# LinXueyuanStdio/LaTeX_OCR

Hardware: NVIDIA H100
Metric: formula-images/sec (train step, 128x512 px, seq<=150) (higher is better)
Workload: dtype bf16

## Files before the change

latex_ocr_b200/csrc/lo_attention.cu:

```cuda
#include <cooperative_groups.h>

#include <mutex>
#include <vector>

#include "lo_common.cuh"
#include "lo_ptx.cuh"

namespace cg = cooperative_groups;

namespace lo {

#ifndef LO_ATT_RPW
#define LO_ATT_RPW 2
#endif
#ifndef LO_ATT_MINB
#define LO_ATT_MINB 2
#endif
#define AP_THREADS 288
#define AP_CWARPS 8
#define AP_STAGES 3
#define AP_MAXSPLIT 16


#ifdef LO_ATT_TIMING
__device__ long long* g_att_ts = nullptr;
__device__ __forceinline__ void att_ts(int k) {
  if (g_att_ts) {
    long long t;
    asm volatile("mov.u64 %0, %%globaltimer;" : "=l"(t));
    g_att_ts[((int64_t)blockIdx.y * gridDim.x + blockIdx.x) * 16 + k] = t;
  }
}
#define ATT_TS(k, cond) do { if (cond) att_ts(k); } while (0)
#else
#define ATT_TS(k, cond) do { } while (0)
#endif

__host__ __device__ __forceinline__ bool att_keep_stage(int i, int depth, int keep_q) {
  const int j = i - depth;
  return j >= 0 && (((j + 1) * keep_q) >> 10) != ((j * keep_q) >> 10);
}

template <int ACT, bool APPROX>
__device__ __forceinline__ float att_act(float x) {
  if constexpr (ACT == 0) return fmaxf(x, 0.f);
  else if constexpr (APPROX) {
    float y;
    asm("tanh.approx.f32 %0, %1;" : "=f"(y) : "f"(x));
    return y;
  } else return tanhf(x);
}
template <int ACT>
__device__ __forceinline__ float att_dact(float pre, float post) {
  if constexpr (ACT == 0) return pre > 0.f ? 1.f : 0.f;
  else return 1.f - post * post;
}

__host__ __device__ __forceinline__ int att_rows_per_split(int R, int nsplit) { return (((R + nsplit - 1) / nsplit) + 1) & ~1; }

template <typename T, int NVA, int NVC>
struct ApCfg {
  static constexpr int CHA = NVA * 256;
  static constexpr int CHC = NVC * 256;
  static constexpr int NVM = NVA > NVC ? NVA : NVC;
  static constexpr int RPW = (sizeof(T) == 2 && NVM <= 2) ? LO_ATT_RPW : 1;
  static constexpr int ROWS = AP_CWARPS * RPW;
  static constexpr int HALF_A = ROWS * CHA;
  static constexpr int HALF_C = ROWS * CHC;
  static constexpr int STAGE_ELEMS = HALF_A + HALF_C;
  static constexpr int STAGE_BYTES = STAGE_ELEMS * (int)sizeof(T);
  static constexpr int SMEM = AP_STAGES * STAGE_BYTES + 128;
};

template <typename T, int NVA, int NVC, bool CL, int ACT, bool MK>
__device__ __forceinline__ void attention_fwd_pipe_cta(
    const T* __restrict__ att1, const T* __restrict__ enc, const float* __restrict__ att2, int64_t att2_stride,
    const float* __restrict__ wf, float* __restrict__ alpha, int64_t alpha_stride, float* __restrict__ ctx,
    float* __restrict__ gate_pre, int64_t gate_stride, float* __restrict__ gctx, bf16* __restrict__ gctx_bf, int R, int nsplit,
    int* __restrict__ counters, float* __restrict__ partials, int keep_q, uint8_t* __restrict__ mask_out, int b, int sp, int64_t g0,
    int64_t pbase) {
  using C = ApCfg<T, NVA, NVC>;
  constexpr int CHA = C::CHA, CHC = C::CHC;
  extern __shared__ __align__(128) uint8_t ap_smem[];
  T* ring = reinterpret_cast<T*>(ap_smem);
  uint64_t* full_bar = reinterpret_cast<uint64_t*>(ap_smem + AP_STAGES * C::STAGE_BYTES);
  uint64_t* empty_bar = full_bar + AP_STAGES;
  float* s_e = reinterpret_cast<float*>(ap_smem + AP_STAGES * C::STAGE_BYTES + 128);
  __shared__ float s_m[AP_CWARPS], s_l[AP_CWARPS];
  __shared__ float s_msplit[AP_MAXSPLIT], s_lsplit[AP_MAXSPLIT];
  __shared__ int s_last;

  const int lane = threadIdx.x & 31, wid = threadIdx.x >> 5;
  const int rps = (R + nsplit - 1) / nsplit;
  const int r0 = sp * rps, r1 = min(R, r0 + rps);
  const int nst = r1 > r0 ? (r1 - r0 + C::ROWS - 1) / C::ROWS : 0;
  const T* a1b = att1 + g0 * CHA;
  const T* eb = enc + g0 * CHC;
  float* alb = alpha + (int64_t)b * alpha_stride;
  ATT_TS(0, threadIdx.x == 0);

  if (threadIdx.x == 0) {
    for (int s = 0; s < AP_STAGES; s++) {
      mbar_init(full_bar + s, 1);
      mbar_init(empty_bar + s, AP_CWARPS);
    }
    fence_barrier_init();
  }
  __syncthreads();
  float m = -INFINITY, l = 0.f;
  float gate_pf = 0.f;
  float acc[NVC * 8];
#pragma unroll
  for (int i = 0; i < NVC * 8; i++) acc[i] = 0.f;

  if (wid == AP_CWARPS) {
    if (lane == 0) {
      const uint64_t pk = l2_policy_evict_normal(), ps = l2_policy_evict_first();
      for (int i = 0; i < nst; i++) {
        const int s = i % AP_STAGES;
        const uint32_t ph = (i / AP_STAGES) & 1;
        mbar_wait(empty_bar + s, ph ^ 1);
        const int row = r0 + i * C::ROWS;
        const int rows = min(C::ROWS, r1 - row);
        const uint32_t bytes_a = (uint32_t)rows * CHA * (uint32_t)sizeof(T), bytes_c = (uint32_t)rows * CHC * (uint32_t)sizeof(T);
        T* sa = ring + (size_t)s * C::STAGE_ELEMS;
        const uint64_t pol = att_keep_stage(i, AP_STAGES, keep_q) ? pk : ps;
        mbar_expect_tx(full_bar + s, bytes_a + bytes_c);
        ATT_TS(6, i == 0);
        ATT_TS(7, i == nst - 1);
        bulk_g2s(sa, a1b + (int64_t)row * CHA, bytes_a, full_bar + s, pol);
        bulk_g2s(sa + C::HALF_A, eb + (int64_t)row * CHC, bytes_c, full_bar + s, pol);
      }
    }
    __syncwarp();
    pdl_wait();
  } else {
    float a2[NVA * 8], wv[NVA * 8];
#pragma unroll
    for (int j = 0; j < NVA; j++) ld8(wf + (j * 32 + lane) * 8, wv + j * 8);
    pdl_wait();
    ATT_TS(1, threadIdx.x == 0);
    pdl_trigger();
#pragma unroll
    for (int j = 0; j < NVA; j++) ld8(att2 + (int64_t)b * att2_stride + (j * 32 + lane) * 8, a2 + j * 8);
    if (CL && gate_pre && (int)threadIdx.x < (CHC + nsplit - 1) / nsplit && sp * ((CHC + nsplit - 1) / nsplit) + (int)threadIdx.x < CHC)
      gate_pf = gate_pre[(int64_t)b * gate_stride + sp * ((CHC + nsplit - 1) / nsplit) + threadIdx.x];
    ATT_TS(2, threadIdx.x == 0);
    for (int i = 0; i < nst; i++) {
      const int s = i % AP_STAGES;
// ... 126 lines not shown
        Lg += ml[1] * scl[q];
      }
    }
    const float invL = 1.0f / Lg;
    const int cps = (CHC + nsplit - 1) / nsplit;
    for (int c = sp * cps + threadIdx.x; c < min(CHC, (sp + 1) * cps); c += AP_THREADS) {
      float t = 0.f;
#pragma unroll
      for (int q = 0; q < 8; q++)
        if (q < nsplit) t = fmaf(cluster.map_shared_rank(s_part, q)[c], scl[q], t);
      t *= invL;
      ctx[(int64_t)b * CHC + c] = t;
      if (gate_pre) {
        const bool pf = c == sp * cps + (int)threadIdx.x && (int)threadIdx.x < AP_CWARPS * 32;
        const float g = sigmoidf_(pf ? gate_pf : gate_pre[(int64_t)b * gate_stride + c]);
        gate_pre[(int64_t)b * gate_stride + c] = g;
        gctx[(int64_t)b * CHC + c] = g * t;
        if (gctx_bf) gctx_bf[(int64_t)b * CHC + c] = __float2bfloat16_rn(g * t);
      } else if (gctx_bf) {
        gctx_bf[(int64_t)b * CHC + c] = __float2bfloat16_rn(t);
      }
    }
    for (int r = r0 + threadIdx.x; r < r1; r += AP_THREADS) alb[r] = expf(s_e[r - r0] - Mg) * invL;
    cluster.sync();
    ATT_TS(5, threadIdx.x == 0);
    return;
  }
  float* part = partials + (pbase + sp) * (CHC + 2);
  for (int c = threadIdx.x; c < CHC; c += AP_THREADS) {
    float t = 0.f;
#pragma unroll
    for (int w = 0; w < AP_CWARPS; w++) t = fmaf(s_acc[w * CHC + c], wsc[w], t);
    part[2 + c] = t;
  }
  if (threadIdx.x == 0) { part[0] = M; part[1] = L; }
  __threadfence();
  __syncthreads();
  if (threadIdx.x == 0) {
    const int ticket = atomicAdd(counters + b, 1);
    s_last = (ticket == nsplit - 1);
    if (s_last) counters[b] = 0;
  }
  __syncthreads();
  if (!s_last) {
    ATT_TS(5, threadIdx.x == 0);
    return;
  }
  __threadfence();
  ATT_TS(9, threadIdx.x == 0);
  const float* pb = partials + pbase * (CHC + 2);
  constexpr int PS = 8;
  constexpr int RB = 4;
  if ((int)threadIdx.x < nsplit) {
    s_msplit[threadIdx.x] = __ldcg(pb + (int64_t)threadIdx.x * (CHC + 2));
    s_lsplit[threadIdx.x] = __ldcg(pb + (int64_t)threadIdx.x * (CHC + 2) + 1);
  }
  float pv[PS], ev[RB];
  auto load_parts = [&](int c) {
#pragma unroll
    for (int s = 0; s < PS; s++) pv[s] = s < nsplit ? __ldcg(pb + (int64_t)s * (CHC + 2) + 2 + c) : 0.f;
  };
  if ((int)threadIdx.x < CHC) load_parts(threadIdx.x);
#pragma unroll
  for (int k = 0; k < RB; k++) {
    const int r = threadIdx.x + k * AP_THREADS;
    ev[k] = r < R ? __ldcg(alb + r) : 0.f;
// ... 24 lines not shown
        const float g = sigmoidf_(gpf[k]);
        gate_pre[(int64_t)b * gate_stride + c] = g;
        gctx[(int64_t)b * CHC + c] = g * t;
        if (gctx_bf) gctx_bf[(int64_t)b * CHC + c] = __float2bfloat16_rn(g * t);
      } else if (gctx_bf) {
        gctx_bf[(int64_t)b * CHC + c] = __float2bfloat16_rn(t);
      }
    }
  }
#pragma unroll
  for (int k = 0; k < RB; k++) {
    const int r = threadIdx.x + k * AP_THREADS;
    if (r < R) alb[r] = expf(ev[k] - Mg) * invL;
  }
  for (int r = threadIdx.x + RB * AP_THREADS; r < R; r += AP_THREADS) alb[r] = expf(__ldcg(alb + r) - Mg) * invL;
  ATT_TS(5, threadIdx.x == 0);
}

template <typename T, int NVA, int NVC, bool CL, int ACT, bool MK>
__global__ void __launch_bounds__(AP_THREADS, LO_ATT_MINB) attention_fwd_pipe_kernel(
    const T* __restrict__ att1, const T* __restrict__ enc, const float* __restrict__ att2, int64_t att2_stride,
    const float* __restrict__ wf, float* __restrict__ alpha, int64_t alpha_stride, float* __restrict__ ctx,
    float* __restrict__ gate_pre, int64_t gate_stride, float* __restrict__ gctx, bf16* __restrict__ gctx_bf, int R, int nsplit,
    int* __restrict__ counters, float* __restrict__ partials, int keep_q, int rpi, uint8_t* __restrict__ mask_out) {
  const int b = blockIdx.y, sp = blockIdx.x;
  attention_fwd_pipe_cta<T, NVA, NVC, CL, ACT, MK>(att1, enc, att2, att2_stride, wf, alpha, alpha_stride, ctx, gate_pre, gate_stride, gctx,
                                                  gctx_bf, R, nsplit, counters, partials, keep_q, mask_out, b, sp,
                                                  (int64_t)(b / rpi) * R, (int64_t)b * nsplit);
}

template <typename T, int NVA, int NVC>
__global__ void __launch_bounds__(AP_THREADS, LO_ATT_MINB) attention_fwd_ragged_kernel(
    const T* __restrict__ att1, const T* __restrict__ enc, const float* __restrict__ att2, int64_t att2_stride,
    const float* __restrict__ wf, float* __restrict__ alpha, int64_t alpha_stride, float* __restrict__ ctx,
    float* __restrict__ gate_pre, int64_t gate_stride, float* __restrict__ gctx, bf16* __restrict__ gctx_bf,
    const int4* __restrict__ cta_map, const int32_t* __restrict__ reg_off, int rpi, int* __restrict__ counters,
    float* __restrict__ partials, int keep_q) {
  const int4 e = cta_map[blockIdx.x];
  const int img = e.x / rpi;
  const int g0 = reg_off[img];
  attention_fwd_pipe_cta<T, NVA, NVC, false, 0, false>(att1, enc, att2, att2_stride, wf, alpha, alpha_stride, ctx, gate_pre, gate_stride,
                                                      gctx, gctx_bf, reg_off[img + 1] - g0, e.z, counters, partials, keep_q, nullptr,
                                                      e.x, e.y, (int64_t)g0, (int64_t)e.w);
}

__host__ __device__ __forceinline__ int att_ragged_row_splits(int ns, int B, int Ri, int64_t sumR, bool fixed) {
  if (fixed) return ns;
  const int64_t q = (int64_t)ns * B * Ri / sumR;
  return q < 1 ? 1 : (q > AP_MAXSPLIT ? AP_MAXSPLIT : (int)q);
}

__global__ void attention_ragged_map_kernel(const int32_t* __restrict__ reg_off, int B, int rpi, int ns, int64_t sumR, int fixed,
                                            int4* __restrict__ cta_map, int* __restrict__ counters) {
  extern __shared__ int s_rows[];
  for (int b = threadIdx.x; b < B; b += blockDim.x) {
    s_rows[b] = att_ragged_row_splits(ns, B, reg_off[b / rpi + 1] - reg_off[b / rpi], sumR, fixed != 0);
    counters[b] = 0;
  }
  __syncthreads();
  if (threadIdx.x == 0) {
    int p = 0;
    for (int b = 0; b < B; b++) {
      s_rows[B + b] = p;
      p += s_rows[b];
    }
  }
// ... 562 lines not shown
  }
  float macc[4][4];
#pragma unroll
  for (int j = 0; j < 4; j++)
#pragma unroll
    for (int i = 0; i < 4; i++) macc[j][i] = 0.f;

  if (wid == AP_CWARPS) {
    const uint64_t pk = l2_policy_evict_normal(), pm = l2_policy_evict_first();
    for (int i = 0; i < nst; i++) {
      const int s = i % ABM_STAGES;
      const uint32_t ph = (i / ABM_STAGES) & 1;
      const int row = r0 + i * ABM_ROWS;
      const int rows = min(ABM_ROWS, r1 - row);
      const uint32_t bytes_m = (uint32_t)((rows + 1) >> 1) * 2u * MB;
      uint8_t* st = ap_smem + (size_t)s * ABM_STAGE_BYTES;
      if (lane == 0) {
        mbar_wait(empty_bar + s, ph ^ 1);
        mbar_expect_tx(full_bar + s, (uint32_t)rows * CH * 2u + bytes_m);
        ATT_TS(6, i == 0);
        ATT_TS(7, i == nst - 1);
      }
      __syncwarp();
      const uint64_t pe = att_keep_stage(i, ABM_STAGES, keep_q) ? pk : pm;
      if (lane < rows) bulk_g2s(st + lane * ABM_PITCH, eb + (int64_t)(row + lane) * CH, CH * 2u, full_bar + s, pe);
      else if (lane == ABM_ROWS) bulk_g2s(st + ABM_ENC_BYTES, mb + (int64_t)(row >> 1) * 2 * MB, bytes_m, full_bar + s, pm);
    }
    __syncwarp();
    pdl_wait();
  } else {
    float sdot = 0.f;
    float gv[16], cxv[16];
#pragma unroll
    for (int j = 0; j < 2; j++) {
      const int c0 = (j * 32 + lane) * 8;
      if (gate) ld8(gate + (int64_t)b * o1_stride + c0, gv + j * 8);
      ld8(ctx + (int64_t)b * CH + c0, cxv + j * 8);
    }
    float gq[4][4];
#pragma unroll
    for (int s = 0; s < 4; s++) {
      const int k0 = 64 * wid + 16 * s + 2 * q;
      if (gate && g < 2) {
        const float2 u = *reinterpret_cast<const float2*>(gate + (int64_t)b * o1_stride + k0);
        const float2 v = *reinterpret_cast<const float2*>(gate + (int64_t)b * o1_stride + k0 + 8);
        gq[s][0] = u.x; gq[s][1] = u.y; gq[s][2] = v.x; gq[s][3] = v.y;
      } else {
// ... 178 lines not shown
      float t = 0.f;
#pragma unroll
      for (int s = 0; s < PS; s++)
        if (s < nsplit) t += pv[s];
      for (int s = PS; s < nsplit; s++) t += __ldcg(pb + (int64_t)s * (CH + 2) + 2 + c);
      if (dwf_part) dwf_part[(int64_t)b * CH + c] = dwf_t[k] + t * a2_t[k];
      datt2[(int64_t)b * dcat_stride + c] = t * wf_t[k];
      if (datt2_bf) datt2_bf[(int64_t)b * dcat_stride + c] = __float2bfloat16_rn(t * wf_t[k]);
    }
  }
  ATT_TS(5, threadIdx.x == 0);
}

int att_pipe_splits(int B, int hint = 0) {
  if (g_opt_att_nsplit > 0) return g_opt_att_nsplit > AP_MAXSPLIT ? AP_MAXSPLIT : g_opt_att_nsplit;
  if (hint > 0) return hint > 8 ? 8 : hint;
  int s = (LO_NUM_SMS * LO_ATT_MINB) / B;
  if (s < 1) s = 1;
  if (s > AP_MAXSPLIT) s = AP_MAXSPLIT;
  if (g_opt_att_cluster && s > 8) s = 8;
  return s;
}

static int att_keep_q(int64_t bytes) {
  static const int64_t l2_bytes = [] {
    int dev = 0, v = 0;
    if (cudaGetDevice(&dev) != cudaSuccess || cudaDeviceGetAttribute(&v, cudaDevAttrL2CacheSize, dev) != cudaSuccess) {
      cudaGetLastError();
      return (int64_t)0;
    }
    return (int64_t)v;
  }();
  int64_t budget = (int64_t)g_opt_att_l2_keep_mb << 20;
  if (budget > l2_bytes) budget = l2_bytes;
  if (budget <= 0 || bytes <= 0) return 0;
  const int64_t q = budget * 1024 / bytes;
  return q > 1024 ? 1024 : (int)q;
}

static cudaAccessPolicyWindow g_att_window{};

static inline bool att_pdl_ok(int abi) { return !abi || g_opt_att_abi_pdl; }

template <typename... KArgs, typename... Args>
static cudaError_t launch_att(void (*kernel)(KArgs...), dim3 grid, size_t smem, int cluster_x, cudaStream_t st, bool pdl, Args... args) {
  cudaLaunchConfig_t cfg{};
  cfg.gridDim = grid;
  cfg.blockDim = dim3(AP_THREADS);
  cfg.dynamicSmemBytes = smem;
  cfg.stream = st;
  cudaLaunchAttribute attr[3];
  int n = 0;
  if (g_att_window.num_bytes) {
    attr[n].id = cudaLaunchAttributeAccessPolicyWindow;
    attr[n].val.accessPolicyWindow = g_att_window;
    n++;
  }
  if (g_opt_pdl && pdl) {
    attr[n].id = cudaLaunchAttributeProgrammaticStreamSerialization;
    attr[n].val.programmaticStreamSerializationAllowed = 1;
// ... 33 lines not shown
  cache.push_back({dev, kernel, smem, per_sm * sms});
  return per_sm * sms;
}

static bool att_grid_cluster(const void* free_kernel, size_t free_smem, int ns, int B, int R) {
  if (!use_cluster(ns, R)) return false;
  if (g_opt_att_cluster != 1) return true;
  return att_resident_ctas(free_kernel, free_smem) < ns * B;
}

template <typename T, int NVA, int NVC, int ACT, bool MK>
static int fwd_launch_m(const AttFwdArgs& x, cudaStream_t st) {
  using C = ApCfg<T, NVA, NVC>;
  constexpr int SM_MAX = C::SMEM + 16 * 1024;
  static bool attr = false;
  if (!attr) {
    LO_CUDA(cudaFuncSetAttribute(attention_fwd_pipe_kernel<T, NVA, NVC, false, ACT, MK>, cudaFuncAttributeMaxDynamicSharedMemorySize, C::SMEM));
    LO_CUDA(cudaFuncSetAttribute(attention_fwd_pipe_kernel<T, NVA, NVC, true, ACT, MK>, cudaFuncAttributeMaxDynamicSharedMemorySize, SM_MAX));
    attr = true;
  }
  const int ns = att_pipe_splits(x.B, x.nsplit_hint);
  const int rpi = x.rows_per_img > 1 ? x.rows_per_img : 1;
  const int keep_q = att_keep_q((int64_t)(x.B / rpi) * x.R * (C::CHA + C::CHC) * (int64_t)sizeof(T));
  if (att_grid_cluster((const void*)attention_fwd_pipe_kernel<T, NVA, NVC, false, ACT, MK>, (size_t)C::SMEM, ns, x.B, x.R)) {
    const size_t smem = C::SMEM + (size_t)((x.R + ns - 1) / ns) * 4;
    LO_CUDA(launch_att(attention_fwd_pipe_kernel<T, NVA, NVC, true, ACT, MK>, dim3(ns, x.B), smem, ns, st, att_pdl_ok(x.abi), (const T*)x.att1, (const T*)x.enc,
                       x.att2, x.att2_stride, x.wf, x.alpha, x.alpha_stride, x.ctx, x.gate_pre, x.gate_stride, x.gctx, x.gctx_bf, x.R, ns,
                       (int*)x.work, (float*)((char*)x.work + 4096), keep_q, rpi, x.mask_out));
  } else {
    LO_CUDA(launch_att(attention_fwd_pipe_kernel<T, NVA, NVC, false, ACT, MK>, dim3(ns, x.B), (size_t)C::SMEM, 1, st, att_pdl_ok(x.abi), (const T*)x.att1,
                       (const T*)x.enc, x.att2, x.att2_stride, x.wf, x.alpha, x.alpha_stride, x.ctx, x.gate_pre, x.gate_stride, x.gctx,
                       x.gctx_bf, x.R, ns, (int*)x.work, (float*)((char*)x.work + 4096), keep_q, rpi, x.mask_out));
  }
  LO_LAUNCH_OK();
  return LO_OK;
}

template <typename T, int NVA, int NVC, int ACT>
static int fwd_launch_a(const AttFwdArgs& x, cudaStream_t st) {
  if constexpr (ACT == 0) {
    if (x.mask_out) return fwd_launch_m<T, NVA, NVC, ACT, true>(x, st);
  }
  return fwd_launch_m<T, NVA, NVC, ACT, false>(x, st);
}

template <typename T, int NVA, int NVC>
static int fwd_launch(const AttFwdArgs& x, cudaStream_t st) {
  return x.act == 1 ? fwd_launch_a<T, NVA, NVC, 1>(x, st) : fwd_launch_a<T, NVA, NVC, 0>(x, st);
}

template <typename T>
static int fwd_dispatch(const AttFwdArgs& x, int C, cudaStream_t st) {
  const int A = x.a_ch > 0 ? x.a_ch : C;
  if (A == 256 && C == 512) return fwd_launch<T, 1, 2>(x, st);
  if (A != C) return fail(LO_EINVAL, "%s: attention width pair (%ld, %ld) not instantiated", __func__, A, C);
// ... 209 lines not shown
```

latex_ocr_b200/csrc/lo_common.cuh:

```cuda
#pragma once
#include <cuda_runtime.h>
#include <cuda_bf16.h>
#include <stdint.h>
#include <stdio.h>
#include <string.h>

#include "../../include/latex_ocr_b200.h"

typedef __nv_bfloat16 bf16;

namespace lo {

extern char g_err[512];
extern int64_t g_launches;

inline int fail(int code, const char* fmt, const char* a = "", long b = 0, long c = 0) {
  snprintf(g_err, sizeof(g_err), fmt, a, b, c);
  return code;
}

#define LO_CHECK_ARG(cond, what)                                                        \
  do {                                                                                  \
    if (!(cond)) return lo::fail(LO_EINVAL, "%s: invalid argument: " what " (line %ld)", __func__, __LINE__); \
  } while (0)
// ... 8 lines not shown
#define LO_LAUNCH_OK()                                                                  \
  do {                                                                                  \
    lo::g_launches++;                                                                   \
    cudaError_t e__ = cudaGetLastError();                                               \
    if (e__ != cudaSuccess)                                                             \
      return lo::fail(LO_ECUDA, "%s: launch failed (%ld) at line %ld", cudaGetErrorString(e__), (long)e__, __LINE__); \
  } while (0)

#define LO_TRY(call)                                                                    \
  do {                                                                                  \
    int r__ = (call);                                                                   \
    if (r__ != LO_OK) return r__;                                                       \
  } while (0)

inline int cdiv(long a, long b) { return (int)((a + b - 1) / b); }

constexpr int LO_NUM_SMS = 132;

#define LO_OPTIONS(X)                                                                                           \
  X(g_opt_att_pipe, "att_pipe", 1)                 \
  X(g_opt_pdl, "pdl", 1)                                                   \
  X(g_opt_att_abi_pdl, "att_abi_pdl", 0)             \
  X(g_opt_att_l2_keep_mb, "att_l2_keep_mb", 24)    \
  X(g_opt_att_nsplit, "att_nsplit", 0)                       \
  X(g_opt_att_cluster, "att_cluster", 1)                      \
  X(g_opt_att_maskbits, "att_maskbits", 1)                 \
  X(g_opt_att_bwd_mma, "att_bwd_mma", 1)                     \
  X(g_opt_dec_streams, "dec_streams", 1)             \
  X(g_opt_dec_fuse, "dec_fuse", 0)                                        \
  X(g_opt_dec_fuse_bwd, "dec_fuse_bwd", 0)                               \
  X(g_opt_dec_cl, "dec_cl", 0)                                                 \
  X(g_opt_dec_cl_bwd, "dec_cl_bwd", 0)                                        \
  X(g_opt_fuse_lstm, "fuse_lstm", 0)                               \
  X(g_opt_skinny_mma, "skinny_mma", 1)                               \
  X(g_opt_skinny_tma, "skinny_tma", 1)                                    \
  X(g_opt_skinny8, "skinny8", 1)                                        \
  X(g_opt_conv_persist, "conv_persist", 1)                      \
  X(g_opt_conv_mt2, "conv_mt2", 1)                            \
  X(g_opt_conv_mc, "conv_mc", 1)                                     \
  X(g_opt_wgrad256, "wgrad256", 0)                                   \
  X(g_opt_det, "deterministic", 0)                                             \
  X(g_opt_dbg_skip, "dbg_skip", 0)                                  \
  X(g_opt_l2_persist_mb, "l2_persist_mb", 0)

#define LO_OPTION_EXTERN(var, name, def) extern int var;
LO_OPTIONS(LO_OPTION_EXTERN)
// ... 138 lines not shown
int gemm(const void* A, int dtA, const void* B, int dtB, void* C, int dtC, const GemmDesc& d, int impl, cudaStream_t st);
int gemm_nt(const void* A, int dtA, int64_t lda, const void* W, int dtW, int64_t ldw, void* C, int dtC, int64_t ldc,
            int M, int N, int K, const float* bias, int accumulate, int relu, int impl, cudaStream_t st);
int gemm_tn(const void* A, int dtA, int64_t lda, const void* B, int dtB, int64_t ldb, void* C, int dtC, int64_t ldc,
            int M, int N, int K, int accumulate, int impl, cudaStream_t st);
int gemm_nn(const void* A, int dtA, int64_t lda, const void* B, int dtB, int64_t ldb, void* C, int dtC, int64_t ldc,
            int M, int N, int K, int accumulate, int impl, cudaStream_t st);
int colsum(const void* X, int dt, float* out, int M, int N, int64_t ld, int accumulate, cudaStream_t st);

struct AttFwdArgs {
  const void *att1, *enc;
  const float* att2; int64_t att2_stride;
  const float* wf;
  float* alpha; int64_t alpha_stride;
  float* ctx; float* gate_pre; int64_t gate_stride; float* gctx; bf16* gctx_bf;
  int B, R;
  void* work;
  int rows_per_img;
  int nsplit_hint;
  int act;
  int a_ch;
  uint8_t* mask_out;
  int abi = 0;
};
struct AttBwdArgs {
  const void *att1, *enc;
  const float *att2, *gate; int64_t o1_stride;
  const float* wf; const float* alpha; int64_t alpha_stride;
  const float* ctx; const float* dgctx; int64_t dg_stride;
  const float* dreg; int64_t dreg_stride; const float* sreg; int64_t sreg_stride;
  float* de; float* datt2; float* dgp; int64_t dcat_stride; bf16* datt2_bf; bf16* dgp_bf; float* dctx_out;
  int B, R;
  void* work;
  float* dwf_part;
  int nsplit_hint;
  int act;
  int a_ch;
  const uint8_t* mask_in;
  int abi = 0;
  void* datt1 = nullptr;
  int ordered_dwf = 0;
};
int attention_fwd_pipe(const AttFwdArgs& x, int dt, int C, cudaStream_t st);
int attention_bwd_pipe(const AttBwdArgs& x, int dt, int C, cudaStream_t st);
struct AttRagged {
  const int32_t* reg_off;
// ... 63 lines not shown
```

latex_ocr_b200/csrc/lo_decoder.cu:

```cuda
#include "lo_common.cuh"
#include "lo_ptx.cuh"

namespace lo {

#define LO_ATT_THREADS 256
#define LO_ATT_WARPS 8
#define LO_ATT_MAXSPLIT 16

static inline int att_splits(int B) {
  int s = (444 + B - 1) / B;
  if (s < 1) s = 1;
  if (s > LO_ATT_MAXSPLIT) s = LO_ATT_MAXSPLIT;
  return s;
}

__device__ __forceinline__ float ldcg_f(const float* p) { return __ldcg(p); }

template <typename T, int NV>
__global__ void __launch_bounds__(LO_ATT_THREADS) attention_fwd_kernel(
    const T* __restrict__ att1, const T* __restrict__ enc, const float* __restrict__ att2, int64_t att2_stride,
    const float* __restrict__ wf, float* __restrict__ alpha, int64_t alpha_stride, float* __restrict__ ctx,
    float* __restrict__ gate_pre, int64_t gate_stride, float* __restrict__ gctx, bf16* __restrict__ gctx_bf, int R, int nsplit,
    int* __restrict__ counters, float* __restrict__ partials, int rpi) {
  constexpr int CH = NV * 256;
// ... 929 lines not shown
    LO_CHECK_ARG(n >= 1 && n <= a->R, "region count of every image in 1..R (reg_off_host)");
  }
  return LO_OK;
}
static int refuse_reg_off(const lo_decoder_args* a) {
  LO_CHECK_ARG(!a->reg_off && !a->reg_off_host, "reg_off / reg_off_host (per-image region counts) are for the decode entry points only");
  return LO_OK;
}
static AttRagged ragged_of(const lo_decoder_args* a) {
  return AttRagged{a->reg_off, a->reg_off_host, (char*)a->work + lo_attention_workspace_bytes(a->B, a->C), 0};
}

static int* work_counters(const lo_decoder_args* a) { return (int*)a->work; }
static inline uint8_t* att_mask_at(const lo_decoder_args* a, int t, int64_t r0) {
  if (!a->att_mask || !g_opt_att_maskbits || !g_opt_att_pipe || a->rows_per_img > 1) return nullptr;
  return a->att_mask + ((int64_t)t * a->B + r0) * ((a->R + 1) & ~1) * (a->A / 8);
}
static float* work_partials(const lo_decoder_args* a) { return (float*)((char*)a->work + 4096); }
static int32_t* work_dlen(const lo_decoder_args* a) { return (int32_t*)((char*)a->work + 2048); }

static int attention_forward_launch(const void* att1, const void* enc, int dt, const float* att2, int64_t att2_stride,
                                    const float* wf, float* alpha, int64_t alpha_stride, float* ctx, float* gate_pre,
                                    int64_t gate_stride, float* gctx, bf16* gctx_bf, int B, int R, int C, void* work, cudaStream_t st,
                                    int rpi = 1, int nsplit_hint = 0, uint8_t* mask_out = nullptr, int abi = 0) {
  if (rpi < 1) rpi = 1;
  if (g_opt_att_pipe) {
    AttFwdArgs x{att1, enc, att2, att2_stride, wf, alpha, alpha_stride, ctx, gate_pre, gate_stride, gctx, gctx_bf, B, R, work, rpi,
                 nsplit_hint, 0, 0, mask_out, abi};
    return attention_fwd_pipe(x, dt, C, st);
  }
  const int ns = att_splits(B);
  int* cnt = (int*)work;
  float* part = (float*)((char*)work + 4096);
  dim3 grid(ns, B);
#define LO_ATT_FWD(T, NV)                                                                                           \
  attention_fwd_kernel<T, NV><<<grid, LO_ATT_THREADS, 0, st>>>((const T*)att1, (const T*)enc, att2, att2_stride, wf, \
                                                               alpha, alpha_stride, ctx, gate_pre, gate_stride, gctx, gctx_bf, R, ns, cnt, part, rpi)
  if (dt == LO_F32) {
    if (C == 256) LO_ATT_FWD(float, 1); else if (C == 512) LO_ATT_FWD(float, 2); else LO_ATT_FWD(float, 4);
  } else {
    if (C == 256) LO_ATT_FWD(bf16, 1); else if (C == 512) LO_ATT_FWD(bf16, 2); else LO_ATT_FWD(bf16, 4);
  }
#undef LO_ATT_FWD
  LO_LAUNCH_OK();
  return LO_OK;
}

static int upload_dlen(const lo_decoder_args* a, cudaStream_t st) {
  int32_t* dl = work_dlen(a);
  LO_CHECK_ARG(a->B <= 512, "B <= 512 (dlen scratch)");
  LO_CUDA(cudaMemsetAsync(dl, 0, (size_t)a->B * 4, st));
// ... 65 lines not shown
    LO_TRY(gemm_nt(a->mean, LO_F32, d.C, a->w_init, dt, d.C, a->hall, LO_F32, d.D, d.B, d.D, d.C, a->b_init, 0, 0, LO_IMPL_SIMT, st));
    LO_TRY(gemm_nt(a->mean, LO_F32, d.C, (const char*)a->w_init + (size_t)d.D * d.C * es, dt, d.C, a->call, LO_F32, d.D, d.B,
                   d.D, d.C, a->b_init + d.D, 0, 0, LO_IMPL_SIMT, st));
  }
  const BfViews bv = bf_views(a, d);
  if (bv.on) {
    LO_TRY(lo_cast(a->hall, LO_F32, bv.hall, LO_BF16, (int64_t)d.B * d.D, (void*)st));
    if ((g_opt_fuse_lstm || g_opt_dec_fuse || g_opt_dec_cl) && d.E % 8 == 0 && d.C % 8 == 0) {
      interleave_wih_kernel<<<LO_NUM_SMS * 2, 256, 0, st>>>((const bf16*)a->w_ih, bv.wil, d.D, d.E, d.C);
      LO_LAUNCH_OK();
    }
  }
  return LO_OK;
}

struct Rows {
  int row0, nrows;
  void* work;
  int nsplit;
  const AttRagged* rg = nullptr;
};

static int forward_step(const lo_decoder_args* a, const Dims& d, int t, const Rows& rs, const int64_t* tok, int64_t tok_stride,
                        float* hd_t, int64_t hd_stride, const float* dmask_t, cudaStream_t st) {
  const int dt = a->dt;
  const int nrows = rs.nrows;
  const int64_t r0 = rs.row0;
  const bool sampling = a->ss_prob && hd_t;
  if (nrows <= 0) return LO_OK;
  const size_t es = dt == LO_F32 ? 4 : 2;
  float* h_prev = a->hall + ((int64_t)t * d.B + r0) * d.D;
  float* c_prev = a->call + ((int64_t)t * d.B + r0) * d.D;
  float* o1 = a->out1 + ((int64_t)t * d.B + r0) * d.O1;
  float* gtmp = a->gtmp + r0 * d.G;
  const int rpi = a->rows_per_img > 1 ? a->rows_per_img : 1;
  const char* att1 = (const char*)a->att1 + (size_t)(r0 / rpi) * d.R * d.A * es;
  const char* enc = (const char*)a->enc + (size_t)(r0 / rpi) * d.R * d.C * es;
  const BfViews bv = bf_views(a, d);
  if (g_opt_dbg_skip & 4) {
  } else if (bv.on && g_opt_skinny_mma && nrows <= 64) {
    LO_TRY(skinny_gemm_nt(bv.hall + ((int64_t)t * d.B + r0) * d.D, d.D, (const bf16*)a->wcat1, d.D, o1, d.O1, nrows, d.O1, d.D, a->bcat1, 1,
                          0, st));
  } else if (bv.on) {
    LO_TRY(tc_gemm_nt_ex(bv.hall + ((int64_t)t * d.B + r0) * d.D, d.D, (const bf16*)a->wcat1, d.D, o1, LO_F32, d.O1, nrows, d.O1, d.D,
                         a->bcat1, 0, 0, 1, 0, 1, st));
  } else {
    LO_TRY(gemm_nt(h_prev, LO_F32, d.D, a->wcat1, dt, d.D, o1, LO_F32, d.O1, nrows, d.O1, d.D, a->bcat1, 0, 0, LO_IMPL_SIMT, st));
  }
  if (rs.rg) {
    if (!(g_opt_dbg_skip & 2)) {
      AttFwdArgs x{a->att1, a->enc, o1, d.O1, a->w_full, a->alphas + t * d.R, (int64_t)d.T * d.R, a->ctx + (int64_t)t * d.B * d.C, o1 + d.A,
                   d.O1, a->gctx + (int64_t)t * d.B * d.C, bv.on ? bv.gctx + (int64_t)t * d.B * d.C : nullptr, nrows, d.R, rs.work,
                   a->rows_per_img, 0, 0, 0, nullptr, 0};
      LO_TRY(attention_fwd_ragged(x, *rs.rg, dt, d.C, st));
    }
  } else if (!(g_opt_dbg_skip & 2))
  LO_TRY(attention_forward_launch(att1, enc, dt, o1, d.O1, a->w_full, a->alphas + (r0 * d.T + t) * d.R, (int64_t)d.T * d.R,
                                  a->ctx + ((int64_t)t * d.B + r0) * d.C, o1 + d.A, d.O1, a->gctx + ((int64_t)t * d.B + r0) * d.C,
                                  bv.on ? bv.gctx + ((int64_t)t * d.B + r0) * d.C : nullptr, nrows, d.R, d.C, rs.work, st,
                                  a->rows_per_img, rs.nsplit, hd_t ? att_mask_at(a, t, r0) : nullptr));
  if (g_opt_dbg_skip & 4) return LO_OK;
  if (bv.on && g_opt_fuse_lstm && !sampling) {
    TcLstmEpi e{a->ptab, tok + r0 * tok_stride, tok_stride, o1 + d.A + d.C, d.O1, c_prev, a->gates + ((int64_t)t * d.B + r0) * d.G,
                a->call + ((int64_t)(t + 1) * d.B + r0) * d.D, a->hall + ((int64_t)(t + 1) * d.B + r0) * d.D,
                bv.hall + ((int64_t)(t + 1) * d.B + r0) * d.D, hd_t ? hd_t + r0 * hd_stride : (float*)nullptr, hd_stride,
                dmask_t ? dmask_t + r0 * hd_stride : (const float*)nullptr, d.D, d.V,
                (const unsigned long long*)((hd_t && a->has_dropout == 2) ? a->dropout_state : nullptr), a->dropout_p, (int)r0, t};
    if (g_opt_skinny_mma && nrows <= 64 && d.C <= 512)
      return skinny_gemm_nt_lstm(bv.gctx + ((int64_t)t * d.B + r0) * d.C, d.C, bv.wil, d.C, nrows, d.D, d.C, e, st);
    return tc_gemm_nt_lstm(bv.gctx + ((int64_t)t * d.B + r0) * d.C, d.C, bv.wil, d.C, nrows, d.D, d.C, e, st);
  }
  if (bv.on && g_opt_skinny_mma && nrows <= 64) {
    LO_TRY(skinny_gemm_nt(bv.gctx + ((int64_t)t * d.B + r0) * d.C, d.C, (const bf16*)a->w_ih + d.E, d.E + d.C, gtmp, d.G, nrows, d.G, d.C,
                          nullptr, 1, 0, st));
  } else if (bv.on) {
    LO_TRY(tc_gemm_nt_ex(bv.gctx + ((int64_t)t * d.B + r0) * d.C, d.C, (const bf16*)a->w_ih + d.E, d.E + d.C, gtmp, LO_F32, d.G, nrows,
                         d.G, d.C, nullptr, 0, 0, 1, 0, 1, st));
  } else {
    LO_TRY(gemm_nt(a->gctx + ((int64_t)t * d.B + r0) * d.C, LO_F32, d.C, (const char*)a->w_ih + (size_t)d.E * es, dt, d.E + d.C, gtmp,
                   LO_F32, d.G, nrows, d.G, d.C, nullptr, 0, 0, LO_IMPL_SIMT, st));
  }
  SsStep ss{};
  if (sampling) {
// ... 257 lines not shown
                                      bvs.gctx + (int64_t)t * d.B * d.C, nrows, d.R, d.C, a->work, st, 1, 0, att_mask_at(a, t, 0)));
      DecStepFwd p{};
      p.gctx = bvs.gctx + (int64_t)t * d.B * d.C; p.ld_gctx = d.C;
      p.wil = bvs.wil; p.ld_wil = d.C;
      const float* dm = (a->has_dropout == 1 && a->dropout_mask) ? a->dropout_mask + (int64_t)t * d.D : nullptr;
      p.e = TcLstmEpi{a->ptab, a->caps + t, a->caps_stride, o1 + d.A + d.C, d.O1, a->call + (int64_t)t * d.B * d.D,
                      a->gates + (int64_t)t * d.B * d.G, a->call + (int64_t)(t + 1) * d.B * d.D, a->hall + (int64_t)(t + 1) * d.B * d.D,
                      bvs.hall + (int64_t)(t + 1) * d.B * d.D, a->hd + (int64_t)t * d.D, (int64_t)d.T * d.D, dm, d.D, d.V,
                      (const unsigned long long*)(a->has_dropout == 2 ? a->dropout_state : nullptr), a->dropout_p, 0, t};
      p.wcat = (const bf16*)a->wcat1; p.ld_wcat = d.D; p.bcat = a->bcat1;
      const bool more = t + 1 < d.T;
      p.o1_next = more ? a->out1 + (int64_t)(t + 1) * d.B * d.O1 : nullptr;
      p.ld_o1 = d.O1; p.N2 = d.O1;
      p.bar = bar; p.bar_target = more ? (++epoch) * (unsigned int)grid : 0u;
      p.M = nrows; p.K = d.C;
      LO_TRY(dec_step_fwd(p, st));
    }
  } else
  for (int chain = 0; chain < nchains; chain++) {
    cudaStream_t cs = chain == 0 ? st : g_side;
    for (int t = 0; t < d.T; t++) {
      const float* dm = (a->has_dropout == 1 && a->dropout_mask) ? a->dropout_mask + (int64_t)t * d.D : nullptr;
      const Rows rs = chain_rows(a, d, chain, nchains, a->bt_host[t]);
      LO_TRY(forward_step(a, d, t, rs, a->caps + t, a->caps_stride, a->hd + (int64_t)t * d.D, (int64_t)d.T * d.D, dm, cs));
    }
  }
  if (nchains == 2) {
    LO_CUDA(cudaEventRecord(g_ev_join, g_side));
    LO_CUDA(cudaStreamWaitEvent(st, g_ev_join, 0));
  }
  }
  if (a->phase == 1) return LO_OK;
  if (g_opt_dbg_skip & 8) return LO_OK;
  const BfViews bvf = bf_views(a, d);
  const bool fc_tc = bvf.on && d.Vl % 64 == 0 && d.D % 64 == 0;
  if (sampling) {
  } else if (fc_tc) {
    LO_TRY(lo_cast(a->hd, LO_F32, bvf.hd, LO_BF16, (int64_t)d.B * d.T * d.D, stream));
    LO_TRY(tc_gemm_nt_ex(bvf.hd, d.D, (const bf16*)a->w_fc, d.D, a->logits, LO_F32, d.Vl, d.B * d.T, d.V, d.D, a->b_fc, 0, 0, 1, 0, 0, st));
  } else {
    LO_TRY(gemm_nt(a->hd, LO_F32, d.D, a->w_fc, a->dt, d.D, a->logits, LO_F32, d.Vl, d.B * d.T, d.V, d.D, a->b_fc, 0, 0, LO_IMPL_SIMT, st));
  }
  if (ragged) {
  }
  if (with_loss) {
    long nvalid = 0;
    for (int t = 0; t < d.T; t++) nvalid += a->bt_host[t];
// ... 507 lines not shown
```

latex_ocr_b200/csrc/lo_ptx.cuh:

```cuda
#pragma once
#include <cuda_runtime.h>
#include <stdint.h>

namespace lo {

__device__ __forceinline__ uint32_t smem_u32(const void* p) { return (uint32_t)__cvta_generic_to_shared(p); }

__device__ __forceinline__ void mbar_init(uint64_t* bar, uint32_t count) {
  asm volatile("mbarrier.init.shared::cta.b64 [%0], %1;" ::"r"(smem_u32(bar)), "r"(count));
}
__device__ __forceinline__ void mbar_expect_tx(uint64_t* bar, uint32_t bytes) {
  asm volatile("mbarrier.arrive.expect_tx.shared::cta.b64 _, [%0], %1;" ::"r"(smem_u32(bar)), "r"(bytes) : "memory");
}
__device__ __forceinline__ uint32_t mbar_try_wait(uint64_t* bar, uint32_t parity) {
  uint32_t done;
  asm volatile(
      "{\n"
      ".reg .pred P1;\n"
      "mbarrier.try_wait.parity.shared::cta.b64 P1, [%1], %2;\n"
      "selp.u32 %0, 1, 0, P1;\n"
      "}\n"
      : "=r"(done)
      : "r"(smem_u32(bar)), "r"(parity)
      : "memory");
  return done;
}
__device__ __forceinline__ void mbar_wait(uint64_t* bar, uint32_t parity) {
  if (mbar_try_wait(bar, parity)) return;
  const long long t0 = clock64();
  while (!mbar_try_wait(bar, parity)) {
    if (clock64() - t0 > 4000000000LL) __trap();
  }
}
__device__ __forceinline__ void fence_barrier_init() { asm volatile("fence.mbarrier_init.release.cluster;" ::: "memory"); }

__device__ __forceinline__ void bulk_g2s(void* dst, const void* src, uint32_t bytes, uint64_t* bar, uint64_t policy) {
  asm volatile(
      "cp.async.bulk.shared::cluster.global.mbarrier::complete_tx::bytes.L2::cache_hint [%0], [%1], %2, [%3], %4;" ::"r"(smem_u32(dst)),
      "l"(reinterpret_cast<uint64_t>(src)), "r"(bytes), "r"(smem_u32(bar)), "l"(policy)
      : "memory");
}
__device__ __forceinline__ uint64_t l2_policy_evict_last() {
  uint64_t p;
  asm volatile("createpolicy.fractional.L2::evict_last.b64 %0, 1.0;" : "=l"(p));
  return p;
}
__device__ __forceinline__ uint64_t l2_policy_evict_first() {
  uint64_t p;
  asm volatile("createpolicy.fractional.L2::evict_first.b64 %0, 1.0;" : "=l"(p));
  return p;
}
__device__ __forceinline__ uint64_t l2_policy_evict_normal() {
  uint64_t p;
  asm volatile("createpolicy.fractional.L2::evict_normal.b64 %0, 1.0;" : "=l"(p));
  return p;
}
__device__ __forceinline__ void mbar_arrive(uint64_t* bar) {
  asm volatile("mbarrier.arrive.shared::cta.b64 _, [%0];" ::"r"(smem_u32(bar)) : "memory");
}

__device__ __forceinline__ void pdl_wait() { asm volatile("griddepcontrol.wait;" ::: "memory"); }
__device__ __forceinline__ void pdl_trigger() { asm volatile("griddepcontrol.launch_dependents;" ::: "memory"); }

// ... 49 lines not shown
```

Before: 2424.

## Prefetch next decoder step's attention stages into L2 at end of attention kernel

At the end of each attention-forward CTA, the producer lane issues bulk L2 prefetches for the encoder/att1 rows that the next timestep will load past the first pipeline stages, bounded by a new L2 prefetch budget option. The L2 keep-policy stage selection is shifted by the prefetched stage count so retained and prefetched regions do not overlap. The host passes the next step's row count so prefetch happens only when the split layout matches. This aims to hide HBM latency at the start of the next step's attention, at the cost of extra L2 traffic and possible eviction of other data.

```diff
diff --git a/latex_ocr_b200/csrc/lo_attention.cu b/latex_ocr_b200/csrc/lo_attention.cu
--- a/latex_ocr_b200/csrc/lo_attention.cu
+++ b/latex_ocr_b200/csrc/lo_attention.cu
@@ -36,8 +36,8 @@
 #define ATT_TS(k, cond) do { } while (0)
 #endif
 
-__host__ __device__ __forceinline__ bool att_keep_stage(int i, int depth, int keep_q) {
-  const int j = i - depth;
+__host__ __device__ __forceinline__ bool att_keep_stage(int i, int depth, int pf, int keep_q) {
+  const int j = i - depth - pf;
   return j >= 0 && (((j + 1) * keep_q) >> 10) != ((j * keep_q) >> 10);
 }
 
@@ -78,7 +78,7 @@
     const float* __restrict__ wf, float* __restrict__ alpha, int64_t alpha_stride, float* __restrict__ ctx,
     float* __restrict__ gate_pre, int64_t gate_stride, float* __restrict__ gctx, bf16* __restrict__ gctx_bf, int R, int nsplit,
     int* __restrict__ counters, float* __restrict__ partials, int keep_q, uint8_t* __restrict__ mask_out, int b, int sp, int64_t g0,
-    int64_t pbase) {
+    int64_t pbase, int pf, bool pf_next) {
   using C = ApCfg<T, NVA, NVC>;
   constexpr int CHA = C::CHA, CHC = C::CHC;
   extern __shared__ __align__(128) uint8_t ap_smem[];
@@ -112,6 +112,15 @@
   float acc[NVC * 8];
 #pragma unroll
   for (int i = 0; i < NVC * 8; i++) acc[i] = 0.f;
+  auto prefetch_next = [&]() {
+    const uint64_t pk = l2_policy_evict_normal();
+    for (int i = AP_STAGES; i < min(nst, AP_STAGES + pf); i++) {
+      const int row = r0 + i * C::ROWS;
+      const int rows = min(C::ROWS, r1 - row);
+      bulk_prefetch_l2(a1b + (int64_t)row * CHA, (uint32_t)rows * CHA * (uint32_t)sizeof(T), pk);
+      bulk_prefetch_l2(eb + (int64_t)row * CHC, (uint32_t)rows * CHC * (uint32_t)sizeof(T), pk);
+    }
+  };
 
   if (wid == AP_CWARPS) {
     if (lane == 0) {
@@ -124,7 +133,7 @@
         const int rows = min(C::ROWS, r1 - row);
         const uint32_t bytes_a = (uint32_t)rows * CHA * (uint32_t)sizeof(T), bytes_c = (uint32_t)rows * CHC * (uint32_t)sizeof(T);
         T* sa = ring + (size_t)s * C::STAGE_ELEMS;
-        const uint64_t pol = att_keep_stage(i, AP_STAGES, keep_q) ? pk : ps;
+        const uint64_t pol = att_keep_stage(i, AP_STAGES, pf, keep_q) ? pk : ps;
         mbar_expect_tx(full_bar + s, bytes_a + bytes_c);
         ATT_TS(6, i == 0);
         ATT_TS(7, i == nst - 1);
@@ -297,6 +306,7 @@
       }
     }
     for (int r = r0 + threadIdx.x; r < r1; r += AP_THREADS) alb[r] = expf(s_e[r - r0] - Mg) * invL;
+    if (pf_next && wid == AP_CWARPS && lane == 0) prefetch_next();
     cluster.sync();
     ATT_TS(5, threadIdx.x == 0);
     return;
@@ -317,6 +327,7 @@
     if (s_last) counters[b] = 0;
   }
   __syncthreads();
+  if (pf_next && wid == AP_CWARPS && lane == 0) prefetch_next();
   if (!s_last) {
     ATT_TS(5, threadIdx.x == 0);
     return;
@@ -387,11 +398,12 @@
     const T* __restrict__ att1, const T* __restrict__ enc, const float* __restrict__ att2, int64_t att2_stride,
     const float* __restrict__ wf, float* __restrict__ alpha, int64_t alpha_stride, float* __restrict__ ctx,
     float* __restrict__ gate_pre, int64_t gate_stride, float* __restrict__ gctx, bf16* __restrict__ gctx_bf, int R, int nsplit,
-    int* __restrict__ counters, float* __restrict__ partials, int keep_q, int rpi, uint8_t* __restrict__ mask_out) {
+    int* __restrict__ counters, float* __restrict__ partials, int keep_q, int rpi, uint8_t* __restrict__ mask_out, int pf,
+    int pf_rows) {
   const int b = blockIdx.y, sp = blockIdx.x;
   attention_fwd_pipe_cta<T, NVA, NVC, CL, ACT, MK>(att1, enc, att2, att2_stride, wf, alpha, alpha_stride, ctx, gate_pre, gate_stride, gctx,
                                                   gctx_bf, R, nsplit, counters, partials, keep_q, mask_out, b, sp,
-                                                  (int64_t)(b / rpi) * R, (int64_t)b * nsplit);
+                                                  (int64_t)(b / rpi) * R, (int64_t)b * nsplit, pf, b < pf_rows && b % rpi == 0);
 }
 
 template <typename T, int NVA, int NVC>
@@ -406,7 +418,7 @@
   const int g0 = reg_off[img];
   attention_fwd_pipe_cta<T, NVA, NVC, false, 0, false>(att1, enc, att2, att2_stride, wf, alpha, alpha_stride, ctx, gate_pre, gate_stride,
                                                       gctx, gctx_bf, reg_off[img + 1] - g0, e.z, counters, partials, keep_q, nullptr,
-                                                      e.x, e.y, (int64_t)g0, (int64_t)e.w);
+                                                      e.x, e.y, (int64_t)g0, (int64_t)e.w, 0, false);
 }
 
 __host__ __device__ __forceinline__ int att_ragged_row_splits(int ns, int B, int Ri, int64_t sumR, bool fixed) {
@@ -1015,7 +1027,7 @@
         ATT_TS(7, i == nst - 1);
       }
       __syncwarp();
-      const uint64_t pe = att_keep_stage(i, ABM_STAGES, keep_q) ? pk : pm;
+      const uint64_t pe = att_keep_stage(i, ABM_STAGES, 0, keep_q) ? pk : pm;
       if (lane < rows) bulk_g2s(st + lane * ABM_PITCH, eb + (int64_t)(row + lane) * CH, CH * 2u, full_bar + s, pe);
       else if (lane == ABM_ROWS) bulk_g2s(st + ABM_ENC_BYTES, mb + (int64_t)(row >> 1) * 2 * MB, bytes_m, full_bar + s, pm);
     }
@@ -1240,7 +1252,7 @@
   return s;
 }
 
-static int att_keep_q(int64_t bytes) {
+static void att_l2_budgets(int64_t& keep, int64_t& prefetch) {
   static const int64_t l2_bytes = [] {
     int dev = 0, v = 0;
     if (cudaGetDevice(&dev) != cudaSuccess || cudaDeviceGetAttribute(&v, cudaDevAttrL2CacheSize, dev) != cudaSuccess) {
@@ -1249,11 +1261,26 @@
     }
     return (int64_t)v;
   }();
-  int64_t budget = (int64_t)g_opt_att_l2_keep_mb << 20;
-  if (budget > l2_bytes) budget = l2_bytes;
+  keep = (int64_t)g_opt_att_l2_keep_mb << 20;
+  keep = keep < 0 ? 0 : (keep > l2_bytes ? l2_bytes : keep);
+  prefetch = (int64_t)g_opt_att_l2_prefetch_mb << 20;
+  prefetch = prefetch < 0 ? 0 : (prefetch > l2_bytes - keep ? l2_bytes - keep : prefetch);
+}
+
+static int att_keep_q(int64_t bytes) {
+  int64_t budget, prefetch;
+  att_l2_budgets(budget, prefetch);
   if (budget <= 0 || bytes <= 0) return 0;
   const int64_t q = budget * 1024 / bytes;
   return q > 1024 ? 1024 : (int)q;
+}
+
+static int att_prefetch_stages(int64_t ctas, int64_t stage_bytes) {
+  int64_t keep, budget;
+  att_l2_budgets(keep, budget);
+  if (budget <= 0 || ctas <= 0) return 0;
+  const int64_t pf = budget / (ctas * stage_bytes);
+  return pf > 4096 ? 4096 : (int)pf;
 }
 
 static cudaAccessPolicyWindow g_att_window{};
@@ -1333,15 +1360,18 @@
   const int ns = att_pipe_splits(x.B, x.nsplit_hint);
   const int rpi = x.rows_per_img > 1 ? x.rows_per_img : 1;
   const int keep_q = att_keep_q((int64_t)(x.B / rpi) * x.R * (C::CHA + C::CHC) * (int64_t)sizeof(T));
+  const bool pf_on = x.pf_rows > 0 && att_pipe_splits(x.pf_rows, x.nsplit_hint) == ns;
+  const int pf = pf_on ? att_prefetch_stages((int64_t)(x.B / rpi) * ns, (int64_t)C::STAGE_BYTES) : 0;
+  const int pf_rows = pf > 0 ? x.pf_rows : 0;
   if (att_grid_cluster((const void*)attention_fwd_pipe_kernel<T, NVA, NVC, false, ACT, MK>, (size_t)C::SMEM, ns, x.B, x.R)) {
     const size_t smem = C::SMEM + (size_t)((x.R + ns - 1) / ns) * 4;
     LO_CUDA(launch_att(attention_fwd_pipe_kernel<T, NVA, NVC, true, ACT, MK>, dim3(ns, x.B), smem, ns, st, att_pdl_ok(x.abi), (const T*)x.att1, (const T*)x.enc,
                        x.att2, x.att2_stride, x.wf, x.alpha, x.alpha_stride, x.ctx, x.gate_pre, x.gate_stride, x.gctx, x.gctx_bf, x.R, ns,
-                       (int*)x.work, (float*)((char*)x.work + 4096), keep_q, rpi, x.mask_out));
+                       (int*)x.work, (float*)((char*)x.work + 4096), keep_q, rpi, x.mask_out, pf, pf_rows));
   } else {
     LO_CUDA(launch_att(attention_fwd_pipe_kernel<T, NVA, NVC, false, ACT, MK>, dim3(ns, x.B), (size_t)C::SMEM, 1, st, att_pdl_ok(x.abi), (const T*)x.att1,
                        (const T*)x.enc, x.att2, x.att2_stride, x.wf, x.alpha, x.alpha_stride, x.ctx, x.gate_pre, x.gate_stride, x.gctx,
-                       x.gctx_bf, x.R, ns, (int*)x.work, (float*)((char*)x.work + 4096), keep_q, rpi, x.mask_out));
+                       x.gctx_bf, x.R, ns, (int*)x.work, (float*)((char*)x.work + 4096), keep_q, rpi, x.mask_out, pf, pf_rows));
   }
   LO_LAUNCH_OK();
   return LO_OK;
diff --git a/latex_ocr_b200/csrc/lo_common.cuh b/latex_ocr_b200/csrc/lo_common.cuh
--- a/latex_ocr_b200/csrc/lo_common.cuh
+++ b/latex_ocr_b200/csrc/lo_common.cuh
@@ -54,6 +54,7 @@
   X(g_opt_pdl, "pdl", 1)                                                   \
   X(g_opt_att_abi_pdl, "att_abi_pdl", 0)             \
   X(g_opt_att_l2_keep_mb, "att_l2_keep_mb", 24)    \
+  X(g_opt_att_l2_prefetch_mb, "att_l2_prefetch_mb", 16)  \
   X(g_opt_att_nsplit, "att_nsplit", 0)                       \
   X(g_opt_att_cluster, "att_cluster", 1)                      \
   X(g_opt_att_maskbits, "att_maskbits", 1)                 \
@@ -238,6 +239,7 @@
   int a_ch;
   uint8_t* mask_out;
   int abi = 0;
+  int pf_rows = 0;
 };
 struct AttBwdArgs {
   const void *att1, *enc;
diff --git a/latex_ocr_b200/csrc/lo_decoder.cu b/latex_ocr_b200/csrc/lo_decoder.cu
--- a/latex_ocr_b200/csrc/lo_decoder.cu
+++ b/latex_ocr_b200/csrc/lo_decoder.cu
@@ -975,11 +975,11 @@
 static int attention_forward_launch(const void* att1, const void* enc, int dt, const float* att2, int64_t att2_stride,
                                     const float* wf, float* alpha, int64_t alpha_stride, float* ctx, float* gate_pre,
                                     int64_t gate_stride, float* gctx, bf16* gctx_bf, int B, int R, int C, void* work, cudaStream_t st,
-                                    int rpi = 1, int nsplit_hint = 0, uint8_t* mask_out = nullptr, int abi = 0) {
+                                    int rpi = 1, int nsplit_hint = 0, uint8_t* mask_out = nullptr, int abi = 0, int pf_rows = 0) {
   if (rpi < 1) rpi = 1;
   if (g_opt_att_pipe) {
     AttFwdArgs x{att1, enc, att2, att2_stride, wf, alpha, alpha_stride, ctx, gate_pre, gate_stride, gctx, gctx_bf, B, R, work, rpi,
-                 nsplit_hint, 0, 0, mask_out, abi};
+                 nsplit_hint, 0, 0, mask_out, abi, pf_rows};
     return attention_fwd_pipe(x, dt, C, st);
   }
   const int ns = att_splits(B);
@@ -1091,7 +1091,7 @@
 };
 
 static int forward_step(const lo_decoder_args* a, const Dims& d, int t, const Rows& rs, const int64_t* tok, int64_t tok_stride,
-                        float* hd_t, int64_t hd_stride, const float* dmask_t, cudaStream_t st) {
+                        float* hd_t, int64_t hd_stride, const float* dmask_t, cudaStream_t st, int next_rows = 0) {
   const int dt = a->dt;
   const int nrows = rs.nrows;
   const int64_t r0 = rs.row0;
@@ -1127,7 +1127,7 @@
   LO_TRY(attention_forward_launch(att1, enc, dt, o1, d.O1, a->w_full, a->alphas + (r0 * d.T + t) * d.R, (int64_t)d.T * d.R,
                                   a->ctx + ((int64_t)t * d.B + r0) * d.C, o1 + d.A, d.O1, a->gctx + ((int64_t)t * d.B + r0) * d.C,
                                   bv.on ? bv.gctx + ((int64_t)t * d.B + r0) * d.C : nullptr, nrows, d.R, d.C, rs.work, st,
-                                  a->rows_per_img, rs.nsplit, hd_t ? att_mask_at(a, t, r0) : nullptr));
+                                  a->rows_per_img, rs.nsplit, hd_t ? att_mask_at(a, t, r0) : nullptr, 0, next_rows));
   if (g_opt_dbg_skip & 4) return LO_OK;
   if (bv.on && g_opt_fuse_lstm && !sampling) {
     TcLstmEpi e{a->ptab, tok + r0 * tok_stride, tok_stride, o1 + d.A + d.C, d.O1, c_prev, a->gates + ((int64_t)t * d.B + r0) * d.G,
@@ -1431,7 +1431,8 @@
     for (int t = 0; t < d.T; t++) {
       const float* dm = (a->has_dropout == 1 && a->dropout_mask) ? a->dropout_mask + (int64_t)t * d.D : nullptr;
       const Rows rs = chain_rows(a, d, chain, nchains, a->bt_host[t]);
-      LO_TRY(forward_step(a, d, t, rs, a->caps + t, a->caps_stride, a->hd + (int64_t)t * d.D, (int64_t)d.T * d.D, dm, cs));
+      const int next_rows = t + 1 < d.T ? chain_rows(a, d, chain, nchains, a->bt_host[t + 1]).nrows : 0;
+      LO_TRY(forward_step(a, d, t, rs, a->caps + t, a->caps_stride, a->hd + (int64_t)t * d.D, (int64_t)d.T * d.D, dm, cs, next_rows));
     }
   }
   if (nchains == 2) {
diff --git a/latex_ocr_b200/csrc/lo_ptx.cuh b/latex_ocr_b200/csrc/lo_ptx.cuh
--- a/latex_ocr_b200/csrc/lo_ptx.cuh
+++ b/latex_ocr_b200/csrc/lo_ptx.cuh
@@ -39,6 +39,11 @@
       "cp.async.bulk.shared::cluster.global.mbarrier::complete_tx::bytes.L2::cache_hint [%0], [%1], %2, [%3], %4;" ::"r"(smem_u32(dst)),
       "l"(reinterpret_cast<uint64_t>(src)), "r"(bytes), "r"(smem_u32(bar)), "l"(policy)
       : "memory");
+}
+__device__ __forceinline__ void bulk_prefetch_l2(const void* src, uint32_t bytes, uint64_t policy) {
+  asm volatile("cp.async.bulk.prefetch.L2.global.L2::cache_hint [%0], %1, %2;" ::"l"(reinterpret_cast<uint64_t>(src)), "r"(bytes),
+               "l"(policy)
+               : "memory");
 }
 __device__ __forceinline__ uint64_t l2_policy_evict_last() {
   uint64_t p;
```

Result: no change. 2437 (median of 6 runs) (+0.5%).
